# turbulencia/tlab

Hardware: AMD Instinct MI355X
Metric: grid-point-updates/s per RK substep (higher is better)
Workload: dtype f64

## Files before the change

### tlab_amd/csrc/capi.cpp

```cpp
#include "../../include/tlab_amd.h"

#include <hip/hip_runtime.h>

#include <cmath>
#include <cstdio>
#include <cstdlib>
#include <cstring>
#include <stdexcept>
#include <string>

#include "internal.hpp"
#include "kernels.hpp"
#include "plan.hpp"

using namespace tlab;

namespace {

thread_local std::string g_err;
hipStream_t g_stream = nullptr;
int g_device = -1;
int g_last_path = 0;
int g_force_path = 0;
DeviceArray *g_ws = nullptr;
// ... 975 lines not shown
    ex.acc = !overwrite;
    ex.fresh_mask = fresh_mask;
    if (tlab_internal_dealiasing()) return false;
    if (ari) {
        if (finish || divx || !tlab_internal_burgers_fusable_anelastic(dir, g, nx, ny, nz)) return false;
        ex.ari = ari; ex.ari_mode = dir == 2 ? 1 : 2; ex.ari_nx = nx; ex.ari_ny = ny;
    }
    ex.nf = nf;
    for (int f = 0; f < nf; ++f) { ex.fs[f] = s[f]; ex.fo[f] = result[f]; ex.fnu[f] = nu[f]; }
    if (finish) {
        if (!tlab_internal_burgers_can_finish(dir, g, nx, ny, nz)) throw Invalid("internal: this Burgers launch cannot finish a field");
        for (int f = 0; f < nf; ++f) ex.ffin[f] = finish[f];
        ex.fdte = dte; ex.fkco = kco; ex.fscale = scale; ex.fny = ny;
        if (clip)
            for (int f = 0; f < nf; ++f)
                if (finish[f] && clip[f]) { ex.fclip[f] = clip[f]; ex.flo[f] = clip_lo[f]; ex.fhi[f] = clip_hi[f]; }
    } else if (clip) {
        for (int f = 0; f < nf; ++f)
            if (clip[f]) throw Invalid("internal: bounds without a finishing launch");
    }
    if (divx) {
        if (!(dir == 1 ? tlab_internal_burgers_can_finish(dir, g, nx, ny, nz) : tlab_internal_burgers_can_div(dir, g, nx, ny, nz)))
            throw Invalid("internal: this Burgers launch cannot write the forcing term");
        ex.fdiv = divx; ex.fidte = idte;
    }
    const bool corr = g->t.der2.need_1der || g->t.der2.direct;
    const int path = choose_path(dir, geom.n, g);
    if (path == PATH_XLINE && !corr) {
        if (fresh_mask) throw Invalid("internal: per-field overwrite is a feature of the y / z tile kernel");
        run_xline(g, geom, MODE_BURGERS, ibc, s[0], vel, result[0], nullptr, nu[0], ex);
    } else if (path == PATH_RTILE && htile_ok(geom.n, MODE_BURGERS)) {
        if (divx && (nf != 1 || s[0] != vel || !tlab_internal_burgers_can_div(dir, g, nx, ny, nz)))
            throw Invalid("internal: the forcing term rides on a one-field launch of the velocity component of that direction");
        run_htile(g, geom, MODE_BURGERS, ibc, s[0], vel, result[0], nullptr, nu[0], ex);
    } else {
        return false;
    }
    g_last_path = path;
    return true;
}

extern "C" {

int tlab_last_kernel_path(void) { return g_last_path; }
int tlab_force_kernel_path(int path) {
    g_force_path = path;
    return TLAB_OK;
}
int tlab_set_tuning(int key, int value) {
    if (key == 1) { rtile_force_chunk(value); return TLAB_OK; }
    if (key == 2) { g_htile_policy = value; return TLAB_OK; }
    if (key == 3 && (value == 16 || value == 32)) { htile_set_lines(value); return TLAB_OK; }
    if (key == 4 && value >= 0) { ptile_set_grid(value); return TLAB_OK; }
    g_err = "tlab_set_tuning: unknown key";
    return TLAB_EINVAL;
}

int tlab_opr_burgers_add(int dir, tlab_fdm_plan_t g, int nx, int ny, int nz, int ibc, double nu, const double *s, const double *vel,
                         double *result, double *tmp1, double *tmp2) {
    return guarded([&] {
        check_common(dir, g, nx, ny, nz, ibc);
        if (!s || !vel || !result || result == s || result == vel) throw Invalid("tlab_opr_burgers_add: null or aliased arrays");
        if (tlab_internal_burgers_acc(dir, g, nx, ny, nz, ibc, nu, s, vel, result)) return;
        if (!tmp1 || !tmp2 || tmp1 == tmp2 || tmp1 == result || tmp2 == result) throw Invalid("tlab_opr_burgers_add: the unfused path needs tmp1, tmp2");
        const int rc = tlab_opr_burgers(dir, g, s == vel ? TLAB_OPR_B_SELF : TLAB_OPR_B_U_IN, nx, ny, nz, ibc, nu, s, vel, tmp1, tmp2, 0);
        if (rc != TLAB_OK) throw Invalid(std::string("tlab_opr_burgers_add: ") + g_err);
        hip_check(launch_add1(result, tmp1, (long long)nx * ny * nz, g_stream), "k_add1");
    });
}

int tlab_opr_burgers_add_n(int dir, tlab_fdm_plan_t g, int nx, int ny, int nz, int ibc, int nf, const double *nu, const double *const *s,
                           const double *vel, double *const *result, double *tmp1, double *tmp2, int overwrite) {
    return guarded([&] {
        check_common(dir, g, nx, ny, nz, ibc);
        if (nf < 1 || nf > 4 || !nu || !s || !vel || !result) throw Invalid("tlab_opr_burgers_add_n: bad arguments (1 to 4 fields)");
        for (int f = 0; f < nf; ++f)
            if (!s[f] || !result[f] || result[f] == s[f] || result[f] == vel) throw Invalid("tlab_opr_burgers_add_n: null or aliased arrays");
        if (!tlab_internal_anelastic() &&
            tlab_internal_burgers_acc_n(dir, g, nx, ny, nz, ibc, nf, nu, s, vel, result, overwrite != 0, nullptr, 0.0, 1.0, 0, nullptr, 0.0, 0u, nullptr, nullptr, nullptr, nullptr)) return;
        for (int f = 0; f < nf; ++f) {
            if (overwrite) hip_check(hipMemsetAsync(result[f], 0, (size_t)nx * ny * nz * sizeof(double), g_stream), "memset");
            const int rc = tlab_opr_burgers_add(dir, g, nx, ny, nz, ibc, nu[f], s[f], vel, result[f], tmp1, tmp2);
            if (rc != TLAB_OK) throw Invalid(std::string("tlab_opr_burgers_add_n: ") + g_err);
        }
    });
}

int tlab_opr_gradient_final(int dir, tlab_fdm_plan_t g, int nx, int ny, int nz, const double *p, double *q, double *h, double dte, double kco,
                            int scale, double *tmp1) {
    return guarded([&] {
        check_common(dir, g, nx, ny, nz, 0);
        if (!p || !q || !h || q == h || p == q || p == h) throw Invalid("tlab_opr_gradient_final: null or aliased arrays");
        if (tlab_internal_gradient_final(dir, g, nx, ny, nz, p, q, h, dte, kco, scale, nullptr, nullptr)) return;
        if (!tmp1 || tmp1 == p || tmp1 == q || tmp1 == h) throw Invalid("tlab_opr_gradient_final: the unfused path needs tmp1");
        const int rc = tlab_opr_partial(dir, g, TLAB_OPR_P1, nx, ny, nz, 0, p, tmp1, nullptr);
        if (rc != TLAB_OK) throw Invalid(std::string("tlab_opr_gradient_final: ") + g_err);
        hip_check(launch_final_update(q, h, tmp1, nullptr, nullptr, dte, kco, scale, nx, ny, nz, g_stream), "k_final_update");
    });
}

int tlab_opr_partial_add(int dir, tlab_fdm_plan_t g, int nx, int ny, int nz, int ibc, const double *u, const double *ub, double scale,
                         double *result, int acc, double *tmp1, double *tmp2) {
    return guarded([&] {
        check_common(dir, g, nx, ny, nz, ibc);
        if (!u || !result || result == u || result == ub) throw Invalid("tlab_opr_partial_add: null or aliased arrays");
        if (tlab_internal_partial_p1_fused(dir, g, nx, ny, nz, ibc, u, ub, scale, result, acc != 0)) return;
// ... 228 lines not shown
```

### tlab_amd/csrc/htile.hip

```cpp
#include <hip/hip_runtime.h>

#include <cstdlib>

#include "device_tables.hpp"
#include "kernels.hpp"
#include "profile.hpp"

namespace tlab {

typedef __attribute__((address_space(1))) char gchar;
typedef __attribute__((address_space(1))) double gdouble;
__device__ __forceinline__ gchar *sgpr_ptr(const void *p) {
    unsigned long long v = (unsigned long long)p;
    asm("" : "+s"(v));
    return (gchar *)v;
}

__device__ __forceinline__ gchar *sgpr_ptr(gchar *p) {
    unsigned long long v = (unsigned long long)p;
    asm("" : "+s"(v));
    return (gchar *)v;
}

__device__ __forceinline__ unsigned vgpr_u32(unsigned v) {
    asm("" : "+v"(v));
    return v;
}

template <bool SYM>
__device__ __forceinline__ double h_stencil(const StencilDev &s, double um3, double um2, double um1, double u0, double up1, double up2,
                                            double up3) {
    if (SYM) return s.c0 * u0 + up1 + um1 + s.c2 * (up2 + um2) + s.c3 * (up3 + um3);
    return up1 - um1 + s.c2 * (up2 - um2);
}
__device__ __forceinline__ double h_dense6(const double (&c)[6], double a0, double a1, double a2, double a3, double a4, double a5) {
    return a0 * c[0] + a1 * c[1] + a2 * c[2] + a3 * c[3] + a4 * c[4] + a5 * c[5];
}

template <int M, int L, bool BAND = false>
__device__ __forceinline__ void h_solve(double (&f)[M], const double *rowtab, const double *ginv, int n, int row0, int c, int C, int l32,
                                        double *s_yl, double *s_r) {
    const double *Lm = rowtab + row0, *Di = rowtab + n + row0, *Cm = rowtab + 2 * n + row0;
    const double *Vt = rowtab + 3 * n + row0, *Wt = rowtab + 4 * n + row0;
    double g = 0.0;
#pragma unroll
    for (int p = 1; p < M; ++p) {
        g = f[p] + Lm[p] * g;
        f[p] = g;
    }
    double yn = 0.0;
#pragma unroll
    for (int p = M - 1; p >= 1; --p) {
        yn = f[p] * Di[p] + Cm[p] * yn;
        f[p] = yn;
    }
    s_yl[c * L + l32] = f[M - 1];
    __syncthreads();
    const int cm = (c + C - 1) % C, cp = (c + 1) % C;
    const double yLprev = s_yl[cm * L + l32];
    s_r[c * L + l32] = f[0] - Lm[0] * yLprev - Cm[0] * f[1];
    __syncthreads();
    double X = 0.0, Xr = 0.0;
    if constexpr (BAND) {
#pragma unroll
        for (int d = 0; d < 5; ++d) {
            X += ginv[c * 5 + d] * s_r[((c + d - 2) & (C - 1)) * L + l32];
            Xr += ginv[cp * 5 + d] * s_r[((cp + d - 2) & (C - 1)) * L + l32];
        }
    } else {
        const double *g0 = ginv + c * C, *g1 = ginv + cp * C;
        for (int q = 0; q < C; ++q) {
            const double rq = s_r[q * L + l32];
            X += g0[q] * rq;
            Xr += g1[q] * rq;
        }
    }
    f[0] = X;
#pragma unroll
    for (int p = 1; p < M; ++p) f[p] = f[p] + Vt[p] * X + Wt[p] * Xr;
}

template <int M, int L, bool BAND = false>
__device__ __forceinline__ void h_solve2(double (&f)[M], double (&h)[M], const double *tf, const double *th, const double *gif, const double *gih, int n,
                                         int row0, int c, int C, int l32, double *s_ylf, double *s_rf, double *s_ylh, double *s_rh) {
    const double *Lf = tf + row0, *Df = tf + n + row0, *Cf = tf + 2 * n + row0, *Vf = tf + 3 * n + row0, *Wf = tf + 4 * n + row0;
    const double *Lh = th + row0, *Dh = th + n + row0, *Ch = th + 2 * n + row0, *Vh = th + 3 * n + row0, *Wh = th + 4 * n + row0;
    double gf = 0.0, gh = 0.0;
#pragma unroll
    for (int p = 1; p < M; ++p) {
        gf = f[p] + Lf[p] * gf;
        gh = h[p] + Lh[p] * gh;
        f[p] = gf;
        h[p] = gh;
    }
    double yf = 0.0, yh = 0.0;
#pragma unroll
    for (int p = M - 1; p >= 1; --p) {
        yf = f[p] * Df[p] + Cf[p] * yf;
        yh = h[p] * Dh[p] + Ch[p] * yh;
        f[p] = yf;
        h[p] = yh;
    }
    s_ylf[c * L + l32] = f[M - 1];
    s_ylh[c * L + l32] = h[M - 1];
    __syncthreads();
    const int cm = (c + C - 1) % C, cp = (c + 1) % C;
    s_rf[c * L + l32] = f[0] - Lf[0] * s_ylf[cm * L + l32] - Cf[0] * f[1];
    s_rh[c * L + l32] = h[0] - Lh[0] * s_ylh[cm * L + l32] - Ch[0] * h[1];
    __syncthreads();
    double Xf = 0.0, Xrf = 0.0, Xh = 0.0, Xrh = 0.0;
    if constexpr (BAND) {
#pragma unroll
        for (int d = 0; d < 5; ++d) {
            const int q0 = ((c + d - 2) & (C - 1)) * L + l32, q1 = ((cp + d - 2) & (C - 1)) * L + l32;
            Xf += gif[c * 5 + d] * s_rf[q0];
            Xrf += gif[cp * 5 + d] * s_rf[q1];
            Xh += gih[c * 5 + d] * s_rh[q0];
            Xrh += gih[cp * 5 + d] * s_rh[q1];
        }
    } else {
        const double *g0f = gif + c * C, *g1f = gif + cp * C, *g0h = gih + c * C, *g1h = gih + cp * C;
        for (int q = 0; q < C; ++q) {
            const double rf = s_rf[q * L + l32], rh = s_rh[q * L + l32];
            Xf += g0f[q] * rf;
            Xrf += g1f[q] * rf;
            Xh += g0h[q] * rh;
            Xrh += g1h[q] * rh;
        }
    }
    f[0] = Xf;
    h[0] = Xh;
#pragma unroll
    for (int p = 1; p < M; ++p) {
        f[p] = f[p] + Vf[p] * Xf + Wf[p] * Xrf;
        h[p] = h[p] + Vh[p] * Xh + Wh[p] * Xrh;
    }
}

template <int M, int MODE, int MAXT, int L, bool DIV = false, int ANEL = 0, bool UNI = false>
__global__ void __launch_bounds__(MAXT, ((L == 16 && MAXT == 256) ? 2 : 1)) k_htile(RTileArgs a) {
    __shared__ double s_yl[32 * L];
    __shared__ double s_r[32 * L];
    __shared__ double s_e[2 * 32 * L];
    __shared__ double s_h[DIV ? 6 * MAXT : 1];
    extern __shared__ double s_tab[];
    constexpr bool NEED1 = (MODE == MODE_P1 || MODE == MODE_P2_P1 || MODE == MODE_BURGERS);
    constexpr bool NEED2 = (MODE != MODE_P1);
    const int l32 = threadIdx.x & (L - 1);
    const int cw = __builtin_amdgcn_readfirstlane((int)(threadIdx.x >> 6)) * (64 / L);
    const int csub = (threadIdx.x & 63) / L;
    const int c = cw + csub;
    const int C = blockDim.x / L;
    const int n = a.g.n;
    const long long rs = a.g.row_stride;
    const bool per = a.s1.periodic != 0;
    const bool corr = !UNI && a.jc.j != nullptr;

    const int tiles_inner = (a.g.lines_inner + L - 1) / L;
    long long tile = blockIdx.x;
    int fi = 0;
    if (MODE == MODE_BURGERS) {
        const long long q = blockIdx.x >> 3;
        fi = (int)(q % a.nf);
        tile = (blockIdx.x & 7) + 8 * (q / a.nf);
        if (tile >= (long long)tiles_inner * (a.g.nlines / a.g.lines_inner)) return;
    }
    const long long outer = tile / tiles_inner;
    const int l0 = (int)(tile % tiles_inner) * L;
    const bool valid = (l0 + l32) < a.g.lines_inner;
    const int lv = valid ? l32 : 0;
    const long long base = outer * a.g.outer_stride + l0 + lv;
    const int row0 = c * M;
    const long long ub = outer * a.g.outer_stride + l0 + (long long)cw * M * rs;
    const unsigned vb = (unsigned)((lv + (long long)csub * M * rs) * 8);
    const long long rs8 = rs * 8;
#define H_ROW0(f) sgpr_ptr((f) + ub)
#define H_NEXT(r) r = sgpr_ptr(r + rs8)
#define H_AT(r) (reinterpret_cast<gdouble *>(r + vgpr_u32(vb)))
    const double *__restrict__ in0 = (MODE == MODE_BURGERS) ? a.fs[fi] : a.in0;
    double *__restrict__ out0 = (MODE == MODE_BURGERS) ? a.fo[fi] : a.out0;
    double nu = (MODE == MODE_BURGERS) ? a.fnu[fi] : a.nu;
    if (ANEL == 2) nu = nu * a.ari[(l0 / a.ari_nx) % a.ari_ny];

    double e[M + 6];
    {
        gchar *r = H_ROW0(in0);
#pragma unroll
        for (int p = 0; p < M; ++p) { e[p + 3] = *H_AT(r); H_NEXT(r); }
    }
#pragma unroll
    for (int k = 0; k < 3; ++k) {
        int rl = row0 - 3 + k, rr = row0 + M + k;
        const bool okl = per || rl >= 0, okr = per || rr < n;
        if (rl < 0) rl += n;
        if (rr >= n) rr -= n;
        e[k] = okl ? in0[base + (long long)rl * rs] : 0.0;
        e[M + 3 + k] = okr ? in0[base + (long long)rr * rs] : 0.0;
    }
    if constexpr (MODE == MODE_P1) {
        if (a.in0b != nullptr) {
            gchar *r = H_ROW0(a.in0b);
#pragma unroll
            for (int p0 = 0; p0 < M; p0 += 8) {
                double t[8];
#pragma unroll
                for (int p = 0; p < 8; ++p) { t[p] = *H_AT(r); H_NEXT(r); }
#pragma unroll
                for (int p = 0; p < 8; ++p) e[p0 + p + 3] = e[p0 + p + 3] + t[p] * a.in0b_scale;
                __builtin_amdgcn_sched_barrier(0);
            }
#pragma unroll
            for (int k = 0; k < 3; ++k) {
                int rl = row0 - 3 + k, rr = row0 + M + k;
                const bool okl = per || rl >= 0, okr = per || rr < n;
                if (rl < 0) rl += n;
                if (rr >= n) rr -= n;
                if (okl) e[k] = e[k] + a.in0b[base + (long long)rl * rs] * a.in0b_scale;
                if (okr) e[M + 3 + k] = e[M + 3 + k] + a.in0b[base + (long long)rr * rs] * a.in0b_scale;
            }
        }
    }


    double *t1 = s_tab, *t2 = s_tab + 5 * n, *gi1 = s_tab + 10 * n, *gi2 = gi1 + C * C, *tj = gi2 + C * C;
    {
        const bool use1 = NEED1 || corr;
        for (int i = threadIdx.x; i < 5 * n; i += blockDim.x) {
            if (use1) t1[i] = a.y1.rowtab[i];
            if (NEED2) t2[i] = a.y2.rowtab[i];
        }
        for (int i = threadIdx.x; i < C * C; i += blockDim.x) {
            if (use1) gi1[i] = a.y1.red[i];
            if (NEED2) gi2[i] = a.y2.red[i];
        }
        if (NEED2 && corr)
            for (int i = threadIdx.x; i < 3 * n; i += blockDim.x) tj[i] = a.jc.j[i];
        if (!UNI && NEED2 && a.s2.rowc != nullptr)
            for (int i = threadIdx.x; i < 5 * n; i += blockDim.x) tj[i] = a.s2.rowc[i];
    }
    __syncthreads();

    double x1[M], x2[NEED2 ? M : 1];
    if (NEED1 || (NEED2 && corr)) {
#pragma unroll
        for (int p = 0; p < M; ++p) x1[p] = h_stencil<false>(a.s1, e[p], e[p + 1], e[p + 2], e[p + 3], e[p + 4], e[p + 5], e[p + 6]);
        if (!UNI && a.s1.rowc != nullptr) {
            const double *rc = a.s1.rowc + row0 * 5;
#pragma unroll
            for (int p = 0; p < M; ++p)
                x1[p] = e[p + 1] * rc[p * 5 + 0] + e[p + 2] * rc[p * 5 + 1] + e[p + 3] * rc[p * 5 + 2] + e[p + 4] * rc[p * 5 + 3] + e[p + 5] * rc[p * 5 + 4];
        }
        if (!per) {
            if (c == 0) {
#pragma unroll
                for (int r = 0; r < 3; ++r) x1[r] = h_dense6(a.s1.bb[r], e[3], e[4], e[5], e[6], e[7], e[8]);
            }
            if (c == C - 1) {
#pragma unroll
                for (int r = 0; r < 3; ++r) x1[M - 3 + r] = h_dense6(a.s1.bt[r], e[M - 3], e[M - 2], e[M - 1], e[M], e[M + 1], e[M + 2]);
            }
        }
    }
    if constexpr (NEED2) {
#pragma unroll
        for (int p = 0; p < M; ++p) x2[p] = h_stencil<true>(a.s2, e[p], e[p + 1], e[p + 2], e[p + 3], e[p + 4], e[p + 5], e[p + 6]);
        if (!UNI && a.s2.rowc != nullptr) {
            const double *rc = tj + row0 * 5;
#pragma unroll
            for (int p = 0; p < M; ++p)
                x2[p] = e[p + 1] * rc[p * 5 + 0] + e[p + 2] * rc[p * 5 + 1] + e[p + 3] * rc[p * 5 + 2] + e[p + 4] * rc[p * 5 + 3] + e[p + 5] * rc[p * 5 + 4];
        }
        if (!per) {
            if (c == 0) {
#pragma unroll
                for (int r = 0; r < 3; ++r) x2[r] = h_dense6(a.s2.bb[r], e[3], e[4], e[5], e[6], e[7], e[8]);
            }
            if (c == C - 1) {
#pragma unroll
                for (int r = 0; r < 3; ++r) x2[M - 3 + r] = h_dense6(a.s2.bt[r], e[M - 3], e[M - 2], e[M - 1], e[M], e[M + 1], e[M + 2]);
            }
        }
    }

    double vl[MODE == MODE_BURGERS ? M : 1];
    if constexpr (MODE == MODE_BURGERS) {
        gchar *r = H_ROW0(a.in2);
#pragma unroll
        for (int p = 0; p < M; ++p) { vl[p] = *H_AT(r); H_NEXT(r); }
    }

    if constexpr (UNI && NEED1 && NEED2) {
        h_solve2<M, L>(x1, x2, t1, t2, gi1, gi2, n, row0, c, C, l32, s_yl, s_r, s_e, s_e + 32 * L);
    } else {
// ... 86 lines not shown
#pragma unroll
            for (int p = 0; p < M; ++p) x2[p] = x1[p] + x2[p];
        }
#pragma unroll
        for (int p = 0; p < M; ++p) { __builtin_nontemporal_store(x2[p], H_AT(ro)); H_NEXT(ro); }
    }
    }
    if constexpr (DIV && MODE == MODE_BURGERS) {
        double tt[M + 6];
#pragma unroll
        for (int p = 0; p < M; ++p) tt[p + 3] = valid ? x2[p] + vl[p] * a.fidte : 0.0;
#pragma unroll
        for (int k = 0; k < 3; ++k) {
            s_h[(c * 6 + k) * L + l32] = tt[3 + k];
            s_h[(c * 6 + 3 + k) * L + l32] = tt[M + k];
        }
        __syncthreads();
        {
            const int cl = (c + C - 1) % C, cr = (c + 1) % C;
            const bool okl = per || c > 0, okr = per || c < C - 1;
#pragma unroll
            for (int k = 0; k < 3; ++k) {
                tt[k] = okl ? s_h[(cl * 6 + 3 + k) * L + l32] : 0.0;
                tt[M + 3 + k] = okr ? s_h[(cr * 6 + k) * L + l32] : 0.0;
            }
        }
        double gg[M];
#pragma unroll
        for (int p = 0; p < M; ++p) gg[p] = h_stencil<false>(a.s1, tt[p], tt[p + 1], tt[p + 2], tt[p + 3], tt[p + 4], tt[p + 5], tt[p + 6]);
        if (!per) {
            if (c == 0) {
#pragma unroll
                for (int r = 0; r < 3; ++r) gg[r] = h_dense6(a.s1.bb[r], tt[3], tt[4], tt[5], tt[6], tt[7], tt[8]);
            }
            if (c == C - 1) {
#pragma unroll
                for (int r = 0; r < 3; ++r) gg[M - 3 + r] = h_dense6(a.s1.bt[r], tt[M - 3], tt[M - 2], tt[M - 1], tt[M], tt[M + 1], tt[M + 2]);
            }
        }
        h_solve<M, L>(gg, t1, gi1, n, row0, c, C, l32, s_yl, s_r);
        if (valid) {
            double fo[M];
            gchar *r = H_ROW0(a.fdiv);
#pragma unroll
            for (int p = 0; p < M; ++p) { fo[p] = *H_AT(r); H_NEXT(r); }
            r = H_ROW0(a.fdiv);
#pragma unroll
            for (int p = 0; p < M; ++p) { *H_AT(r) = fo[p] + gg[p]; H_NEXT(r); }
        }
    }
#undef H_AT
#undef H_NEXT
#undef H_ROW0
}


template <int M, int L, int C, bool DIV = false, bool BAND = false>
__global__ void __launch_bounds__(L * C, 1) k_ptile(RTileArgs a, long long nitems) {
    constexpr int N = M * C;
    constexpr int GI = BAND ? 5 * C : C * C;
    __shared__ double s_sep[4 * C * L];
    __shared__ double s_t[2 * 3 * 5 * M];
    __shared__ double s_gi[2 * GI];
    extern __shared__ double s_op[];
    const int l32 = threadIdx.x & (L - 1);
    const int wv = __builtin_amdgcn_readfirstlane((int)(threadIdx.x >> 6));
    const int cw = wv * (64 / L);
    const int csub = (threadIdx.x & 63) / L;
    const int c = cw + csub;
    const long long rs = a.g.row_stride;
    const long long rs8 = rs * 8;
    const bool per = a.s1.periodic != 0;
    const int tiles_inner = a.g.lines_inner / L;
    const long long ntiles = (long long)tiles_inner * (a.g.nlines / a.g.lines_inner);

    for (int i = threadIdx.x; i < 2 * 3 * 5 * M; i += blockDim.x) {
        const int sys = i / (15 * M), v = (i / (5 * M)) % 3, arr = (i / M) % 5, p = i % M;
        const int chunk = v == 0 ? 0 : (v == 1 ? 1 : C - 1);
        s_t[i] = (sys == 0 ? a.y1.rowtab : a.y2.rowtab)[arr * N + chunk * M + p];
    }
    for (int i = threadIdx.x; i < GI; i += blockDim.x) {
        s_gi[i] = BAND ? a.y1.band[i] : a.y1.red[i];
        s_gi[GI + i] = BAND ? a.y2.band[i] : a.y2.red[i];
    }
    const int var = (c == 0) ? 0 : (c == C - 1 ? 2 : 1);
    const double *t1 = s_t + var * 5 * M, *t2 = s_t + (3 + var) * 5 * M;

    auto decode = [&](long long it, long long &tile, int &fi) {
        const long long q = it >> 3;
        fi = (int)(q % a.nf);
        tile = (it & 7) + 8 * (q / a.nf);
    };
    constexpr int PR = L / 2, RI = 64 / PR, RW = N / (L * C / 64), NI = RW / RI;
    const unsigned lane = threadIdx.x & 63;
    const unsigned dma_voff = (unsigned)(((long long)(lane / PR) * rs + (lane % PR) * 2) * 8);
    const unsigned lds_base = (unsigned)(unsigned long long)s_op;
    auto prefetch = [&](long long it) {
        long long tile;
        int fi;
        decode(it, tile, fi);
        if (tile >= ntiles) return;
        const long long outer = tile / tiles_inner;
        const int l0 = (int)(tile % tiles_inner) * L;
        gchar *src = sgpr_ptr(a.fs[fi] + outer * a.g.outer_stride + l0 + (long long)(RW * wv) * rs);
        unsigned dst = lds_base + (unsigned)(RW * wv) * (L * 8);
        const long long step = RI * rs8;
// ... 101 lines not shown
            double tt[M + 6];
#pragma unroll
            for (int p = 0; p < M; ++p) tt[p + 3] = x2[p] + vl[p] * a.fidte;
            const int cl = (c + C - 1) % C, cr = (c + 1) % C;
            const bool okl = per || c > 0, okr = per || c < C - 1;
            __syncthreads();
#pragma unroll
            for (int k = 0; k < 3; ++k) s_sep[(c * 3 + k) * L + l32] = tt[3 + k];
            __syncthreads();
#pragma unroll
            for (int k = 0; k < 3; ++k) tt[M + 3 + k] = okr ? s_sep[(cr * 3 + k) * L + l32] : 0.0;
            __syncthreads();
#pragma unroll
            for (int k = 0; k < 3; ++k) s_sep[(c * 3 + k) * L + l32] = tt[M + k];
            __syncthreads();
#pragma unroll
            for (int k = 0; k < 3; ++k) tt[k] = okl ? s_sep[(cl * 3 + k) * L + l32] : 0.0;
            __syncthreads();
            double gg[M];
#pragma unroll
            for (int p = 0; p < M; ++p) gg[p] = h_stencil<false>(a.s1, tt[p], tt[p + 1], tt[p + 2], tt[p + 3], tt[p + 4], tt[p + 5], tt[p + 6]);
            if (!per) {
                if (c == 0) {
#pragma unroll
                    for (int r = 0; r < 3; ++r) gg[r] = h_dense6(a.s1.bb[r], tt[3], tt[4], tt[5], tt[6], tt[7], tt[8]);
                }
                if (c == C - 1) {
#pragma unroll
                    for (int r = 0; r < 3; ++r) gg[M - 3 + r] = h_dense6(a.s1.bt[r], tt[M - 3], tt[M - 2], tt[M - 1], tt[M], tt[M + 1], tt[M + 2]);
                }
            }
            h_solve<M, L, BAND>(gg, t1, s_gi, M, 0, c, C, l32, s_sep, s_sep + C * L);
            double fo[M];
            gchar *r = H_ROW0(a.fdiv);
#pragma unroll
            for (int p = 0; p < M; ++p) { fo[p] = *H_AT(r); H_NEXT(r); }
            r = H_ROW0(a.fdiv);
            asm volatile("s_waitcnt vmcnt(0)" ::: "memory");
#pragma unroll
            for (int p = 0; p < M; ++p) { *H_AT(r) = fo[p] + gg[p]; H_NEXT(r); }
        }
#undef H_AT
#undef H_NEXT
#undef H_ROW0
        __syncthreads();
    }
}

static int g_htile_persist = [] { const char *e = getenv("TLAB_HTILE_PERSIST"); return (e && atoi(e) == 0) ? 0 : 1; }();
static int g_ptile_band = [] { const char *e = getenv("TLAB_PTILE_BAND"); return e ? atoi(e) : 1; }();
static int g_ncu = 0;
static int g_ptile_grid = 0;
void ptile_set_grid(int n) { g_ptile_grid = n > 0 ? n : 0; }
static long long ptile_cus() {
    if (g_ptile_grid) return g_ptile_grid;
    if (!g_ncu) {
        int dev = 0;
        hipDeviceProp_t pr;
        if (hipGetDevice(&dev) == hipSuccess && hipGetDeviceProperties(&pr, dev) == hipSuccess) g_ncu = pr.multiProcessorCount;
        if (g_ncu <= 0) g_ncu = 256;
        g_ncu = g_ncu >= 8 ? (g_ncu / 8) * 8 : 8;
    }
    return g_ncu;
}
static bool ptile_ok(const RTileArgs &a, int L, int C) {
    if (!g_htile_persist || a.g.lines_inner % L != 0 || !a.y1.chunk_invariant || !a.y2.chunk_invariant) return false;
    if (L == 32 && C == 16 && a.g.n == 512) return true;
    static const bool long_ok = [] { const char *e = getenv("TLAB_PTILE_1024"); return !(e && atoi(e) == 0); }();
    return long_ok && L == 16 && C == 32 && a.g.n == 1024 && a.y1.band != nullptr && a.y2.band != nullptr;
}
static int g_htile_uni = [] { const char *e = getenv("TLAB_HTILE_UNI"); return (e && atoi(e) == 0) ? 0 : 1; }();
static int g_htile_lines = [] { const char *e = getenv("TLAB_HTILE_LINES"); return (e && atoi(e) == 16) ? 16 : 32; }();
void htile_set_lines(int lines) { g_htile_lines = lines; }
bool htile_narrow() { return g_htile_lines == 16; }

int htile_chunk(int n, int mode) {
    const bool two = (mode == MODE_P2_P1 || mode == MODE_BURGERS);
    auto ok = [&](int m, int cmax) { return n % m == 0 && (n / m) % 2 == 0 && n / m <= cmax; };
    if (two) {
        if (ok(32, 16)) return 32;
        if (ok(16, 16)) return 16;
        if (n == 1024) return 32;
        return 0;
    }
    if (ok(32, 32)) return 32;
    if (ok(64, 16)) return 64;
    if (ok(16, 32)) return 16;
    return 0;
}

template <int M, int MAXT, int L = 32>
static hipError_t launch_htile_m(int mode, int C, long long tiles, const RTileArgs &a, hipStream_t st) {
    const long long nwg = (mode == MODE_BURGERS) ? 8LL * a.nf * ((tiles + 7) / 8) : tiles;
    const dim3 grid((unsigned)nwg), block(L * C);
    const size_t lds = ((size_t)(a.s2.rowc ? 15 : 13) * a.g.n + (size_t)2 * C * C) * sizeof(double);
    const double pts = (double)a.g.nlines * a.g.n;
    const char *name = mode == MODE_P1 ? "k_htile<P1>" : mode == MODE_P2 ? "k_htile<P2>" : mode == MODE_P2_P1 ? "k_htile<P2_P1>" :
                       a.fdiv ? "k_htile<BURGERS+div>" : "k_htile<BURGERS>";
    const double bpp = (mode == MODE_P1 || mode == MODE_P2) ? 16 : 24;
    double bytes = pts * (bpp + (a.acc ? 8 : 0));
    if (mode == MODE_P1) bytes += pts * ((a.in0b ? 8 : 0) + (a.fq ? 24 : 0));
    if (mode == MODE_BURGERS) {
        bytes = pts * 8;
        for (int f = 0; f < a.nf; ++f) bytes += pts * ((a.fs[f] == a.in2 ? 0 : 8) + 8 + ((a.acc && !((a.fresh_mask >> f) & 1u)) ? 8 : 0));
        if (a.fdiv) bytes += pts * 16;
    }
    const bool uni = g_htile_uni && a.jc.j == nullptr && a.s1.rowc == nullptr && a.s2.rowc == nullptr;
    if constexpr (M == 32 && MAXT == 512)
        if (mode == MODE_BURGERS && uni && !a.ari && ptile_ok(a, L, C) && (!a.fdiv || (a.nf == 1 && a.fs[0] == a.in2)))
            name = a.fdiv ? "k_ptile<BURGERS+div>" : "k_ptile<BURGERS>";
    ProfScope ps(name, st, bytes);
    switch (mode) {
    case MODE_P1: hipLaunchKernelGGL((k_htile<M, MODE_P1, MAXT, L>), grid, block, lds, st, a); break;
    case MODE_P2: hipLaunchKernelGGL((k_htile<M, MODE_P2, MAXT, L>), grid, block, lds, st, a); break;
    case MODE_P2_P1: hipLaunchKernelGGL((k_htile<M, MODE_P2_P1, MAXT, L>), grid, block, lds, st, a); break;
    case MODE_BURGERS:
        if (a.fdiv) {
            if constexpr (M == 32 && MAXT == 512) {
                if (a.nf != 1 || a.fs[0] != a.in2 || C * L > MAXT || a.s1.rowc != nullptr || a.ari) return hipErrorInvalidValue;
                if (uni && ptile_ok(a, L, C)) {
                    const unsigned pg = (unsigned)(nwg < ptile_cus() ? nwg : ptile_cus());
                    if constexpr (L == 32) {
                        if (g_ptile_band == 2 && a.y1.band && a.y2.band) hipLaunchKernelGGL((k_ptile<32, 32, 16, true, true>), dim3(pg), dim3(512), (size_t)a.g.n * 32 * sizeof(double), st, a, nwg);
                        else hipLaunchKernelGGL((k_ptile<32, 32, 16, true>), dim3(pg), dim3(512), (size_t)a.g.n * 32 * sizeof(double), st, a, nwg);
                    }
                    else hipLaunchKernelGGL((k_ptile<32, 16, 32, true, true>), dim3(pg), dim3(512), (size_t)a.g.n * 16 * sizeof(double), st, a, nwg);
                } else if (uni) hipLaunchKernelGGL((k_htile<M, MODE_BURGERS, MAXT, L, true, 0, true>), grid, block, lds, st, a);
                else hipLaunchKernelGGL((k_htile<M, MODE_BURGERS, MAXT, L, true>), grid, block, lds, st, a);
            } else {
                return hipErrorInvalidValue;
            }
        } else if (a.ari) {
            if constexpr (M == 32 && MAXT == 512 && L == 32) {
                if (a.ari_mode == 1) hipLaunchKernelGGL((k_htile<M, MODE_BURGERS, MAXT, L, false, 1>), grid, block, lds, st, a);
                else if (a.ari_mode == 2 && a.ari_nx % L == 0) hipLaunchKernelGGL((k_htile<M, MODE_BURGERS, MAXT, L, false, 2>), grid, block, lds, st, a);
                else return hipErrorInvalidValue;
            } else {
                return hipErrorInvalidValue;
            }
        } else {
            if constexpr (M == 32 && MAXT == 512) {
                if (uni && ptile_ok(a, L, C)) {
                    const unsigned pg = (unsigned)(nwg < ptile_cus() ? nwg : ptile_cus());
                    if constexpr (L == 32) {
                        if (g_ptile_band && a.y1.band && a.y2.band) hipLaunchKernelGGL((k_ptile<32, 32, 16, false, true>), dim3(pg), dim3(512), (size_t)a.g.n * 32 * sizeof(double), st, a, nwg);
                        else hipLaunchKernelGGL((k_ptile<32, 32, 16>), dim3(pg), dim3(512), (size_t)a.g.n * 32 * sizeof(double), st, a, nwg);
                    }
                    else hipLaunchKernelGGL((k_ptile<32, 16, 32, false, true>), dim3(pg), dim3(512), (size_t)a.g.n * 16 * sizeof(double), st, a, nwg);
                } else if (uni) hipLaunchKernelGGL((k_htile<M, MODE_BURGERS, MAXT, L, false, 0, true>), grid, block, lds, st, a);
                else hipLaunchKernelGGL((k_htile<M, MODE_BURGERS, MAXT, L>), grid, block, lds, st, a);
            } else {
                hipLaunchKernelGGL((k_htile<M, MODE_BURGERS, MAXT, L>), grid, block, lds, st, a);
            }
        }
        break;
    default: return hipErrorInvalidValue;
    }
    return hipGetLastError();
}

hipError_t launch_htile(int mode, const RTileArgs &a, hipStream_t st) {
    const int n = a.g.n;
    const int M = htile_chunk(n, mode);
    if (M == 0) return hipErrorInvalidValue;
    const int C = n / M;
    if (C & 1) return hipErrorInvalidValue;
    if ((double)(64 / 16 - 1) * M * (double)a.g.row_stride * 8.0 + 512.0 >= 4294967296.0) return hipErrorInvalidValue;
    const bool two = (mode == MODE_P2_P1 || mode == MODE_BURGERS);
    const bool narrow = (g_htile_lines == 16) && mode == MODE_BURGERS && M == 32 && C <= 16;
    const bool long16 = two && M == 32 && C == 32;
    const int L = (narrow || long16) ? 16 : 32;
    const long long tiles_inner = (a.g.lines_inner + L - 1) / L;
    const long long tiles = tiles_inner * (a.g.nlines / a.g.lines_inner);
    if (narrow) return launch_htile_m<32, 256, 16>(mode, C, tiles, a, st);
    if (long16) return launch_htile_m<32, 512, 16>(mode, C, tiles, a, st);
    if (M == 64) return launch_htile_m<64, 512>(mode, C, tiles, a, st);
    if (M == 32) return (C <= 16) ? launch_htile_m<32, 512>(mode, C, tiles, a, st) : launch_htile_m<32, 1024>(mode, C, tiles, a, st);
    return (C <= 16) ? launch_htile_m<16, 512>(mode, C, tiles, a, st) : launch_htile_m<16, 1024>(mode, C, tiles, a, st);
}

}
```

### tlab_amd/csrc/kernels.hpp

```cpp
#pragma once
#include <hip/hip_runtime.h>

#include <vector>

#include "device_tables.hpp"

namespace tlab {

struct XLineArgs {
    const double *in0;
    const double *in1;
    double *out0, *out1;
    const double *in0b;
    double in0b_scale;
    int acc;
    long long nlines;
    StencilDev s1, s2;
    SystemDev y1, y2;
    double nu;
    int nf;
    const double *fs[4];
    double *fo[4];
    double fnu[4];
    double *fq;
// ... 41 lines not shown
    int ari_mode, ari_nx, ari_ny;
};

struct GenericArgs {
    const double *in0;
    const double *in1;
    double *out0;
    LineGeom g;
    StencilDev s;
    SystemDev y;
    JacCorrDev jc;
};

struct PentaArgs {
    const double *in0;
    double *out0;
    LineGeom g;
    const double *rhs;
    const double *lu;
    int periodic, ibc;
    double rb[4 * 8];
    double rt[5 * 7];
};
hipError_t launch_penta1(const PentaArgs &a, hipStream_t st);

struct PentaTileArgs {
    const double *in0;
    double *out0;
    LineGeom g;
    const double *rhs;
    const double *rows;
    const double *blocks;
    const double *smw;
    double r6, r7;
    int periodic, ibc;
    double rb[4 * 8];
    double rt[5 * 7];
};
bool pentatile_ok(const LineGeom &g);
void pentatile_build(int n, int C, bool periodic, int ibc, const double *lu, std::vector<double> &rows, std::vector<double> &blocks, std::vector<double> &smw);
hipError_t launch_pentatile(const PentaTileArgs &a, hipStream_t st);
bool pentatile_x_ok(const LineGeom &g);
hipError_t launch_pentatile_x(const PentaTileArgs &a, hipStream_t st);

bool xline_supported(int n);
int rtile_chunk(int n);
void rtile_force_chunk(int m);
hipError_t launch_xline(int mode, int n, int chunks, bool lane_variant, const XLineArgs &a, hipStream_t st);
hipError_t launch_rtile(int mode, const RTileArgs &a, hipStream_t st);
int htile_chunk(int n, int mode);
void ptile_set_grid(int n);
void htile_set_lines(int lines);
bool htile_narrow();
hipError_t launch_htile(int mode, const RTileArgs &a, hipStream_t st);
hipError_t launch_generic(bool sym, const GenericArgs &a, hipStream_t st);
hipError_t launch_burgers_epilogue(double *out, const double *vel, const double *d1, double nu, long long ntot, hipStream_t st);
hipError_t launch_fill(double *out, double v, long long ntot, hipStream_t st);
hipError_t launch_transpose(const double *a, double *b, int nra, int nca, hipStream_t st);

hipError_t launch_add3(double *h, const double *a, const double *b, const double *c, long long n, hipStream_t st);
hipError_t launch_axpy3(double *o1, double *o2, double *o3, const double *h1, const double *h2, const double *h3, const double *q1,
                        const double *q2, const double *q3, double s, long long n, hipStream_t st);
hipError_t launch_axpy3w(double *o1, double *o2, double *o3, const double *h1, const double *h2, const double *h3, const double *q1,
                         const double *q2, const double *q3, double s, const double *w, int nx, int ny, long long n, hipStream_t st);
hipError_t launch_minmax_partial(const double *a, const double *v, const double *w, const double *odx, const double *ody, const double *odz,
                                 int mode, int nx, int ny, int nz, int koff, int zon, double *part, int nblocks, hipStream_t st);
hipError_t launch_negate(double *a, long long n, hipStream_t st);
hipError_t launch_scale(double *a, double alpha, long long n, hipStream_t st);
hipError_t launch_surface_flux(double *ref, const double *t, int j, int javg, double sign, double diff, double cpl, double *avg_scratch, int nx, int ny,
                               int nz, hipStream_t st);
hipError_t launch_weight_y(double *out, const double *in, const double *w, int nx, int ny, long long n, int mode, hipStream_t st);
hipError_t launch_burgers_epilogue_anelastic(double *out, const double *vel, const double *d1, double nu, const double *ri, int nx, int ny,
                                             long long n, hipStream_t st);
hipError_t launch_pencil_repack(double *a, double *buf, int nxh, int ny, int kmax, int nproc, const int *ioff, const long long *base, int dir,
                                hipStream_t st);
hipError_t launch_add1(double *h, const double *a, long long n, hipStream_t st);
hipError_t launch_axpy1(double *o, const double *a, const double *b, double s, long long n, hipStream_t st);
hipError_t launch_sum3(double *a, const double *b, const double *c, long long n, hipStream_t st);
hipError_t launch_sub3(double *h1, double *h2, double *h3, const double *a, const double *b, const double *c, long long n, hipStream_t st);

hipError_t launch_get_wall_planes(const double *f, double *hb, double *ht, int nx, int ny, int nz, hipStream_t st);
hipError_t launch_fill_wall_planes(double *f, double vb, double vt, int nx, int ny, int nz, hipStream_t st);
struct ClipBounds { double lo, hi; };
hipError_t launch_final_update(double *q, double *h, const double *g, const double *pb, const double *pt, double dte, double kco, int scale,
                               int nx, int ny, int nz, hipStream_t st, const double *gw = nullptr, const ClipBounds *clip = nullptr);
hipError_t launch_clip(double *a, double lo, double hi, long long n, hipStream_t st);
hipError_t launch_rk_update(double *q, double *h, double dte, double kco, int scale, long long n, hipStream_t st, const ClipBounds *clip = nullptr);
hipError_t launch_set_wall_planes(double *f, const double *pb, const double *pt, int nx, int ny, int nz, hipStream_t st);
hipError_t launch_buffer_relax(int nf, double *const *h, const double *const *a, const double *ref, const double *tau, int nx, int ny, int nz,
                               int offset, int size, hipStream_t st);
hipError_t launch_buffer_relax_plane(int nf, double *const *h, double *const *s, const double *ref, const double *tau, const double *const *bc,
                                     const ClipBounds *const *clip, double dte, double kco, int scale, int nx, int ny, int nz, int offset, int size,
                                     int jloc, hipStream_t st);
constexpr int BODY_FORCE_MAX_SCAL = 6;
struct BodyForce {
    int cor = 0, bod = 0, ns = 0;
    double f[3] = {0, 0, 0}, g[3] = {0, 0, 0}, c[BODY_FORCE_MAX_SCAL] = {0, 0, 0, 0, 0, 0}, geo_u = 0.0, geo_w = 0.0;
    int sidx[BODY_FORCE_MAX_SCAL] = {0, 1, 2, 3, 4, 5};
    bool any() const { return (cor == 1 && (f[0] != 0.0 || f[1] != 0.0 || f[2] != 0.0)) || (cor == 2 && f[1] != 0.0) || (bod != 0 && (g[0] != 0.0 || g[1] != 0.0 || g[2] != 0.0)); }
};
hipError_t launch_body_force(const BodyForce &F, double *const *hq, const double *const *q, const double *const *s, const double *prof, int nx, int ny,
                             int nz, hipStream_t st);
hipError_t launch_airwater_linear(double *l, const double *s1, const double *s2, int ns, double p1, double p2, double pd, long long n, hipStream_t st);

struct InfraredCoef { double rb[3][4], rt[2][4], l0[3]; };
struct DerTables;
// ... 23 lines not shown
```

Before: 8.650 billion.

## Make htile kernel persistent with one-time table staging and optional LDS halo exchange

Turns the htile kernel into a grid-stride persistent kernel. By default the grid is sized from occupancy times the CU count, so the coefficient tables are staged into LDS once per block instead of once per tile. It also sizes dynamic LDS to the systems each mode actually uses, and adds an optional halo path (off by default). That path exchanges chunk-boundary rows via wave shuffles and shared memory instead of re-reading them from global memory. The persistent loop adds a barrier per iteration and adds register pressure from reloading the kernel arguments.

```diff
diff --git a/tlab_amd/csrc/capi.cpp b/tlab_amd/csrc/capi.cpp
--- a/tlab_amd/csrc/capi.cpp
+++ b/tlab_amd/csrc/capi.cpp
@@ -1051,6 +1051,8 @@
     if (key == 2) { g_htile_policy = value; return TLAB_OK; }
     if (key == 3 && (value == 16 || value == 32)) { htile_set_lines(value); return TLAB_OK; }
     if (key == 4 && value >= 0) { ptile_set_grid(value); return TLAB_OK; }
+    if (key == 5 && (value == 0 || value == 1)) { htile_set_halo(value); return TLAB_OK; }
+    if (key == 6 && value >= -1) { htile_set_grid(value); return TLAB_OK; }
     g_err = "tlab_set_tuning: unknown key";
     return TLAB_EINVAL;
 }
diff --git a/tlab_amd/csrc/htile.hip b/tlab_amd/csrc/htile.hip
--- a/tlab_amd/csrc/htile.hip
+++ b/tlab_amd/csrc/htile.hip
@@ -1,6 +1,8 @@
 #include <hip/hip_runtime.h>
 
 #include <cstdlib>
+#include <map>
+#include <tuple>
 
 #include "device_tables.hpp"
 #include "kernels.hpp"
@@ -22,18 +24,26 @@
     return (gchar *)v;
 }
 
+typedef __attribute__((address_space(4))) RTileArgs KArgs;
+__device__ __forceinline__ const KArgs *opaque_args(const KArgs *p) {
+    unsigned long long v = (unsigned long long)p;
+    asm volatile("" : "+s"(v));
+    return (const KArgs *)v;
+}
+
 __device__ __forceinline__ unsigned vgpr_u32(unsigned v) {
     asm("" : "+v"(v));
     return v;
 }
 
-template <bool SYM>
-__device__ __forceinline__ double h_stencil(const StencilDev &s, double um3, double um2, double um1, double u0, double up1, double up2,
+template <bool SYM, class S>
+__device__ __forceinline__ double h_stencil(const S &s, double um3, double um2, double um1, double u0, double up1, double up2,
                                             double up3) {
     if (SYM) return s.c0 * u0 + up1 + um1 + s.c2 * (up2 + um2) + s.c3 * (up3 + um3);
     return up1 - um1 + s.c2 * (up2 - um2);
 }
-__device__ __forceinline__ double h_dense6(const double (&c)[6], double a0, double a1, double a2, double a3, double a4, double a5) {
+template <class A>
+__device__ __forceinline__ double h_dense6(const A &c, double a0, double a1, double a2, double a3, double a4, double a5) {
     return a0 * c[0] + a1 * c[1] + a2 * c[2] + a3 * c[3] + a4 * c[4] + a5 * c[5];
 }
 
@@ -137,18 +147,31 @@
     }
 }
 
+constexpr bool htile_stays(int M, int mode, int maxt) { return maxt <= 512 && M <= 32 && mode != MODE_P2; }
+
 template <int M, int MODE, int MAXT, int L, bool DIV = false, int ANEL = 0, bool UNI = false>
-__global__ void __launch_bounds__(MAXT, ((L == 16 && MAXT == 256) ? 2 : 1)) k_htile(RTileArgs a) {
-    __shared__ double s_yl[32 * L];
-    __shared__ double s_r[32 * L];
-    __shared__ double s_e[2 * 32 * L];
+__global__ void __launch_bounds__(MAXT, ((L == 16 && MAXT == 256) ? 2 : 1)) k_htile(RTileArgs a, int halo, long long nitems) {
+    __shared__ double s_all[4 * 32 * L];
+    double *const s_yl = s_all, *const s_e = s_all + 32 * L, *const s_r = s_all + 3 * 32 * L;
     __shared__ double s_h[DIV ? 6 * MAXT : 1];
     extern __shared__ double s_tab[];
     constexpr bool NEED1 = (MODE == MODE_P1 || MODE == MODE_P2_P1 || MODE == MODE_BURGERS);
     constexpr bool NEED2 = (MODE != MODE_P1);
-    const int l32 = threadIdx.x & (L - 1);
-    const int cw = __builtin_amdgcn_readfirstlane((int)(threadIdx.x >> 6)) * (64 / L);
-    const int csub = (threadIdx.x & 63) / L;
+    constexpr bool DUAL = UNI && NEED1 && NEED2;
+    constexpr int NS = 64 / L;
+    constexpr bool STAY = htile_stays(M, MODE, MAXT);
+    constexpr int HX0 = (DUAL ? 2 : 1) * 32 * L;
+    static_assert(6 * L * ((MAXT + 63) / 64) <= 4 * 32 * L - HX0, "halo rows of every wave edge must fit into the free part of the separator arrays");
+    double *const hx = s_all + HX0;
+    bool staged = false;
+    const KArgs *const ka = (const KArgs *)__builtin_amdgcn_kernarg_segment_ptr();
+    for (long long item = blockIdx.x; item < nitems; item += gridDim.x) {
+    const KArgs &a = *opaque_args(ka);
+    unsigned tx = threadIdx.x;
+    asm volatile("" : "+v"(tx));
+    const int l32 = tx & (L - 1);
+    const int cw = __builtin_amdgcn_readfirstlane((int)(tx >> 6)) * (64 / L);
+    const int csub = (tx & 63) / L;
     const int c = cw + csub;
     const int C = blockDim.x / L;
     const int n = a.g.n;
@@ -157,23 +180,29 @@
     const bool corr = !UNI && a.jc.j != nullptr;
 
     const int tiles_inner = (a.g.lines_inner + L - 1) / L;
-    long long tile = blockIdx.x;
+    const int row0 = c * M;
+    const long long rs8 = rs * 8;
+    const bool hfirst = (csub == 0), hlast = (csub == NS - 1) || (c == C - 1);
+    double *const t1 = s_tab, *const t2 = t1 + ((NEED1 || corr) ? 5 * n : 0), *const gi1 = t2 + (NEED2 ? 5 * n : 0);
+    double *const gi2 = gi1 + ((NEED1 || corr) ? C * C : 0), *const tj = gi2 + (NEED2 ? C * C : 0);
+    long long tile = item;
     int fi = 0;
     if (MODE == MODE_BURGERS) {
-        const long long q = blockIdx.x >> 3;
+        const long long q = item >> 3;
         fi = (int)(q % a.nf);
-        tile = (blockIdx.x & 7) + 8 * (q / a.nf);
-        if (tile >= (long long)tiles_inner * (a.g.nlines / a.g.lines_inner)) return;
+        tile = (item & 7) + 8 * (q / a.nf);
+        if (tile >= (long long)tiles_inner * (a.g.nlines / a.g.lines_inner)) {
+            if constexpr (STAY) continue;
+            else return;
+        }
     }
     const long long outer = tile / tiles_inner;
     const int l0 = (int)(tile % tiles_inner) * L;
     const bool valid = (l0 + l32) < a.g.lines_inner;
     const int lv = valid ? l32 : 0;
     const long long base = outer * a.g.outer_stride + l0 + lv;
-    const int row0 = c * M;
     const long long ub = outer * a.g.outer_stride + l0 + (long long)cw * M * rs;
     const unsigned vb = (unsigned)((lv + (long long)csub * M * rs) * 8);
-    const long long rs8 = rs * 8;
 #define H_ROW0(f) sgpr_ptr((f) + ub)
 #define H_NEXT(r) r = sgpr_ptr(r + rs8)
 #define H_AT(r) (reinterpret_cast<gdouble *>(r + vgpr_u32(vb)))
@@ -188,14 +217,16 @@
 #pragma unroll
         for (int p = 0; p < M; ++p) { e[p + 3] = *H_AT(r); H_NEXT(r); }
     }
-#pragma unroll
-    for (int k = 0; k < 3; ++k) {
-        int rl = row0 - 3 + k, rr = row0 + M + k;
-        const bool okl = per || rl >= 0, okr = per || rr < n;
-        if (rl < 0) rl += n;
-        if (rr >= n) rr -= n;
-        e[k] = okl ? in0[base + (long long)rl * rs] : 0.0;
-        e[M + 3 + k] = okr ? in0[base + (long long)rr * rs] : 0.0;
+    if (!halo) {
+#pragma unroll
+        for (int k = 0; k < 3; ++k) {
+            int rl = row0 - 3 + k, rr = row0 + M + k;
+            const bool okl = per || rl >= 0, okr = per || rr < n;
+            if (rl < 0) rl += n;
+            if (rr >= n) rr -= n;
+            e[k] = okl ? in0[base + (long long)rl * rs] : 0.0;
+            e[M + 3 + k] = okr ? in0[base + (long long)rr * rs] : 0.0;
+        }
     }
     if constexpr (MODE == MODE_P1) {
         if (a.in0b != nullptr) {
@@ -209,21 +240,23 @@
                 for (int p = 0; p < 8; ++p) e[p0 + p + 3] = e[p0 + p + 3] + t[p] * a.in0b_scale;
                 __builtin_amdgcn_sched_barrier(0);
             }
-#pragma unroll
-            for (int k = 0; k < 3; ++k) {
-                int rl = row0 - 3 + k, rr = row0 + M + k;
-                const bool okl = per || rl >= 0, okr = per || rr < n;
-                if (rl < 0) rl += n;
-                if (rr >= n) rr -= n;
-                if (okl) e[k] = e[k] + a.in0b[base + (long long)rl * rs] * a.in0b_scale;
-                if (okr) e[M + 3 + k] = e[M + 3 + k] + a.in0b[base + (long long)rr * rs] * a.in0b_scale;
-            }
-        }
-    }
-
-
-    double *t1 = s_tab, *t2 = s_tab + 5 * n, *gi1 = s_tab + 10 * n, *gi2 = gi1 + C * C, *tj = gi2 + C * C;
-    {
+            if (!halo) {
+#pragma unroll
+                for (int k = 0; k < 3; ++k) {
+                    int rl = row0 - 3 + k, rr = row0 + M + k;
+                    const bool okl = per || rl >= 0, okr = per || rr < n;
+                    if (rl < 0) rl += n;
+                    if (rr >= n) rr -= n;
+                    if (okl) e[k] = e[k] + a.in0b[base + (long long)rl * rs] * a.in0b_scale;
+                    if (okr) e[M + 3 + k] = e[M + 3 + k] + a.in0b[base + (long long)rr * rs] * a.in0b_scale;
+                }
+            }
+        }
+    }
+
+    const bool first = !staged;
+    if (first) {
+        staged = true;
         const bool use1 = NEED1 || corr;
         for (int i = threadIdx.x; i < 5 * n; i += blockDim.x) {
             if (use1) t1[i] = a.y1.rowtab[i];
@@ -238,7 +271,43 @@
         if (!UNI && NEED2 && a.s2.rowc != nullptr)
             for (int i = threadIdx.x; i < 5 * n; i += blockDim.x) tj[i] = a.s2.rowc[i];
     }
-    __syncthreads();
+    if (halo) {
+        const int wv = cw / NS;
+        if (hfirst) {
+#pragma unroll
+            for (int k = 0; k < 3; ++k) hx[((2 * wv + 0) * 3 + k) * L + l32] = e[3 + k];
+        }
+        if (hlast) {
+#pragma unroll
+            for (int k = 0; k < 3; ++k) hx[((2 * wv + 1) * 3 + k) * L + l32] = e[M + k];
+        }
+#pragma unroll
+        for (int k = 0; k < 3; ++k) {
+            if constexpr (NS == 2) {
+                const double t = __shfl_xor(hfirst ? e[M + k] : e[3 + k], 32);
+                if (hfirst) e[M + 3 + k] = t;
+                else e[k] = t;
+            } else {
+                const double dn = __shfl_up(e[M + k], L), up = __shfl_down(e[3 + k], L);
+                if (!hfirst) e[k] = dn;
+                if (!hlast) e[M + 3 + k] = up;
+            }
+        }
+    }
+    if (first || halo) __syncthreads();
+    if (halo) {
+        const int cl = (c + C - 1) % C, cr = (c + 1) % C;
+        if (hfirst) {
+            const bool okl = per || c > 0;
+#pragma unroll
+            for (int k = 0; k < 3; ++k) e[k] = okl ? hx[((2 * (cl / NS) + 1) * 3 + k) * L + l32] : 0.0;
+        }
+        if (hlast) {
+            const bool okr = per || c < C - 1;
+#pragma unroll
+            for (int k = 0; k < 3; ++k) e[M + 3 + k] = okr ? hx[((2 * (cr / NS) + 0) * 3 + k) * L + l32] : 0.0;
+        }
+    }
 
     double x1[M], x2[NEED2 ? M : 1];
     if (NEED1 || (NEED2 && corr)) {
@@ -431,6 +500,9 @@
 #undef H_AT
 #undef H_NEXT
 #undef H_ROW0
+    if constexpr (!STAY) break;
+    if (item + gridDim.x < nitems) __syncthreads();
+    }
 }
 
 
@@ -638,8 +710,7 @@
 static int g_ncu = 0;
 static int g_ptile_grid = 0;
 void ptile_set_grid(int n) { g_ptile_grid = n > 0 ? n : 0; }
-static long long ptile_cus() {
-    if (g_ptile_grid) return g_ptile_grid;
+static long long device_cus() {
     if (!g_ncu) {
         int dev = 0;
         hipDeviceProp_t pr;
@@ -649,6 +720,7 @@
     }
     return g_ncu;
 }
+static long long ptile_cus() { return g_ptile_grid ? g_ptile_grid : device_cus(); }
 static bool ptile_ok(const RTileArgs &a, int L, int C) {
     if (!g_htile_persist || a.g.lines_inner % L != 0 || !a.y1.chunk_invariant || !a.y2.chunk_invariant) return false;
     if (L == 32 && C == 16 && a.g.n == 512) return true;
@@ -659,6 +731,26 @@
 static int g_htile_lines = [] { const char *e = getenv("TLAB_HTILE_LINES"); return (e && atoi(e) == 16) ? 16 : 32; }();
 void htile_set_lines(int lines) { g_htile_lines = lines; }
 bool htile_narrow() { return g_htile_lines == 16; }
+static int g_htile_halo = [] { const char *e = getenv("TLAB_HTILE_HALO"); return (e && atoi(e) == 1) ? 1 : 0; }();
+void htile_set_halo(int on) { g_htile_halo = on ? 1 : 0; }
+static int g_htile_grid = [] { const char *e = getenv("TLAB_HTILE_STAY"); return (e && atoi(e) == 0) ? -1 : 0; }();
+void htile_set_grid(int n) { g_htile_grid = n < 0 ? -1 : n; }
+static long long htile_grid(const void *kern, int threads, size_t lds, long long nitems) {
+    if (g_htile_grid < 0) return nitems;
+    long long g = g_htile_grid;
+    if (g == 0) {
+        static std::map<std::tuple<const void *, int, size_t>, int> occ;
+        const auto key = std::make_tuple(kern, threads, lds);
+        auto it = occ.find(key);
+        if (it == occ.end()) {
+            int nb = 0;
+            if (hipOccupancyMaxActiveBlocksPerMultiprocessor(&nb, kern, threads, lds) != hipSuccess || nb < 1) nb = 1;
+            it = occ.emplace(key, nb).first;
+        }
+        g = device_cus() * it->second;
+    }
+    return g < nitems ? g : nitems;
+}
 
 int htile_chunk(int n, int mode) {
     const bool two = (mode == MODE_P2_P1 || mode == MODE_BURGERS);
@@ -678,8 +770,14 @@
 template <int M, int MAXT, int L = 32>
 static hipError_t launch_htile_m(int mode, int C, long long tiles, const RTileArgs &a, hipStream_t st) {
     const long long nwg = (mode == MODE_BURGERS) ? 8LL * a.nf * ((tiles + 7) / 8) : tiles;
-    const dim3 grid((unsigned)nwg), block(L * C);
-    const size_t lds = ((size_t)(a.s2.rowc ? 15 : 13) * a.g.n + (size_t)2 * C * C) * sizeof(double);
+    const dim3 block(L * C);
+    const bool use1 = mode != MODE_P2 || a.jc.j != nullptr, use2 = mode != MODE_P1;
+    const size_t sys = (size_t)5 * a.g.n + (size_t)C * C;
+    const size_t lds = ((use1 ? sys : 0) + (use2 ? sys + (size_t)(a.s2.rowc ? 5 : a.jc.j ? 3 : 0) * a.g.n : 0)) * sizeof(double);
+    auto go = [&](void (*kern)(RTileArgs, int, long long)) {
+        const long long g = htile_stays(M, mode, MAXT) ? htile_grid((const void *)kern, L * C, lds, nwg) : nwg;
+        hipLaunchKernelGGL(kern, dim3((unsigned)g), block, lds, st, a, g_htile_halo, nwg);
+    };
     const double pts = (double)a.g.nlines * a.g.n;
     const char *name = mode == MODE_P1 ? "k_htile<P1>" : mode == MODE_P2 ? "k_htile<P2>" : mode == MODE_P2_P1 ? "k_htile<P2_P1>" :
                        a.fdiv ? "k_htile<BURGERS+div>" : "k_htile<BURGERS>";
@@ -697,9 +795,9 @@
             name = a.fdiv ? "k_ptile<BURGERS+div>" : "k_ptile<BURGERS>";
     ProfScope ps(name, st, bytes);
     switch (mode) {
-    case MODE_P1: hipLaunchKernelGGL((k_htile<M, MODE_P1, MAXT, L>), grid, block, lds, st, a); break;
-    case MODE_P2: hipLaunchKernelGGL((k_htile<M, MODE_P2, MAXT, L>), grid, block, lds, st, a); break;
-    case MODE_P2_P1: hipLaunchKernelGGL((k_htile<M, MODE_P2_P1, MAXT, L>), grid, block, lds, st, a); break;
+    case MODE_P1: go(k_htile<M, MODE_P1, MAXT, L>); break;
+    case MODE_P2: go(k_htile<M, MODE_P2, MAXT, L>); break;
+    case MODE_P2_P1: go(k_htile<M, MODE_P2_P1, MAXT, L>); break;
     case MODE_BURGERS:
         if (a.fdiv) {
             if constexpr (M == 32 && MAXT == 512) {
@@ -711,15 +809,15 @@
                         else hipLaunchKernelGGL((k_ptile<32, 32, 16, true>), dim3(pg), dim3(512), (size_t)a.g.n * 32 * sizeof(double), st, a, nwg);
                     }
                     else hipLaunchKernelGGL((k_ptile<32, 16, 32, true, true>), dim3(pg), dim3(512), (size_t)a.g.n * 16 * sizeof(double), st, a, nwg);
-                } else if (uni) hipLaunchKernelGGL((k_htile<M, MODE_BURGERS, MAXT, L, true, 0, true>), grid, block, lds, st, a);
-                else hipLaunchKernelGGL((k_htile<M, MODE_BURGERS, MAXT, L, true>), grid, block, lds, st, a);
+                } else if (uni) go(k_htile<M, MODE_BURGERS, MAXT, L, true, 0, true>);
+                else go(k_htile<M, MODE_BURGERS, MAXT, L, true>);
             } else {
                 return hipErrorInvalidValue;
             }
         } else if (a.ari) {
             if constexpr (M == 32 && MAXT == 512 && L == 32) {
-                if (a.ari_mode == 1) hipLaunchKernelGGL((k_htile<M, MODE_BURGERS, MAXT, L, false, 1>), grid, block, lds, st, a);
-                else if (a.ari_mode == 2 && a.ari_nx % L == 0) hipLaunchKernelGGL((k_htile<M, MODE_BURGERS, MAXT, L, false, 2>), grid, block, lds, st, a);
+                if (a.ari_mode == 1) go(k_htile<M, MODE_BURGERS, MAXT, L, false, 1>);
+                else if (a.ari_mode == 2 && a.ari_nx % L == 0) go(k_htile<M, MODE_BURGERS, MAXT, L, false, 2>);
                 else return hipErrorInvalidValue;
             } else {
                 return hipErrorInvalidValue;
@@ -733,10 +831,10 @@
                         else hipLaunchKernelGGL((k_ptile<32, 32, 16>), dim3(pg), dim3(512), (size_t)a.g.n * 32 * sizeof(double), st, a, nwg);
                     }
                     else hipLaunchKernelGGL((k_ptile<32, 16, 32, false, true>), dim3(pg), dim3(512), (size_t)a.g.n * 16 * sizeof(double), st, a, nwg);
-                } else if (uni) hipLaunchKernelGGL((k_htile<M, MODE_BURGERS, MAXT, L, false, 0, true>), grid, block, lds, st, a);
-                else hipLaunchKernelGGL((k_htile<M, MODE_BURGERS, MAXT, L>), grid, block, lds, st, a);
+                } else if (uni) go(k_htile<M, MODE_BURGERS, MAXT, L, false, 0, true>);
+                else go(k_htile<M, MODE_BURGERS, MAXT, L>);
             } else {
-                hipLaunchKernelGGL((k_htile<M, MODE_BURGERS, MAXT, L>), grid, block, lds, st, a);
+                go(k_htile<M, MODE_BURGERS, MAXT, L>);
             }
         }
         break;
diff --git a/tlab_amd/csrc/kernels.hpp b/tlab_amd/csrc/kernels.hpp
--- a/tlab_amd/csrc/kernels.hpp
+++ b/tlab_amd/csrc/kernels.hpp
@@ -117,6 +117,8 @@
 void ptile_set_grid(int n);
 void htile_set_lines(int lines);
 bool htile_narrow();
+void htile_set_halo(int on);
+void htile_set_grid(int n);
 hipError_t launch_htile(int mode, const RTileArgs &a, hipStream_t st);
 hipError_t launch_generic(bool sym, const GenericArgs &a, hipStream_t st);
 hipError_t launch_burgers_epilogue(double *out, const double *vel, const double *d1, double nu, long long ntot, hipStream_t st);
```

New measurement: 8.698 billion, median of 6. No clear change (+0.6%).
